# Alisah-Ozcan/HEonGPU

Hardware: AMD Instinct MI355X
Metric: homomorphic mults/sec (CKKS N=2^16, L=16) + NTT GB/s vs HBM roofline (higher is better)
Workload: dtype u64

## Files before the change

heongpu_amd/csrc/ntt.hip:

```cpp
#include "ntt.hpp"
#define HEGPU_FP_TU ntt
#include "fpmod.cuh"

namespace hegpu {

#define NTT_THREADS 256

#ifdef NTT_ABLATION_HEADER
#include NTT_ABLATION_HEADER
#else
__device__ __forceinline__ u64 gld(const u64* p) { return *p; }
__device__ __forceinline__ void gst(u64* p, u64 v) { *p = v; }
#define NTT_ABLATE_BFLY(x, y, w)
#define NTT_ABLATE_FPBFLY(x, y, w)
#define NTT_ABLATE_TW(load, root0, s) (load)
#define NTT_FP_TW(t, i, c) ((t)[i])
#endif

__device__ __forceinline__ u64 csub(u64 x, u64 m) { return (x >= m) ? x - m : x; }

typedef unsigned long long u64x2_t __attribute__((ext_vector_type(2)));
struct ConstTw {
    const u64x2_t __attribute__((address_space(4)))* p;
    __device__ __forceinline__ ulonglong2 operator[](u32 i) const
// ... 618 lines not shown
    for (int k = 0; k < 8; k++)
        *reinterpret_cast<ulonglong2*>(&lds[row_phys(row * 256 + 16 * i0 + 2 * k)]) =
            make_ulonglong2(x[2 * k], x[2 * k + 1]);
    wave_lds_fence();
    row_store_all(a, ps, md, a.out + ps.out_off, (u64) blockIdx.x * 4096 + row * 256 + i0, lds, row, i0);
}

__device__ __forceinline__ void fwd_row_body_fp(const NttArgs& a, const PolySel& ps, const Mod& md, u64* lds)
{
    const int t = threadIdx.x;
    const FC fc = make_fc(md.q, FP_SITE(FPS_FWD_ROW, a.n_power - 12));
    const int s1 = a.n_power - 8;
    const ulonglong2* __restrict__ tw = a.tw + ((u64) ps.mod << a.n_power);
    u64* __restrict__ p = a.out + ps.out_off + (u64) blockIdx.x * 4096;

    const int row = t >> 4, i0 = t & 15;
    const u32 crow = blockIdx.x * 16 + row;
    double x[16];
#pragma unroll
    for (int k = 0; k < 16; k++) x[k] = as_f64(p[row * 256 + i0 + 16 * k]);
    fp_ct_radix<4>(x, tw, (1u << s1) + crow, fc, 0u, true);
#pragma unroll
    for (int k = 0; k < 16; k++) lds[row_phys(row * 256 + i0 + 16 * k)] = as_bits(x[k]);
    wave_lds_fence();
#pragma unroll
    for (int k = 0; k < 8; k++) {
        ulonglong2 v = *reinterpret_cast<const ulonglong2*>(&lds[row_phys(row * 256 + 16 * i0 + 2 * k)]);
        x[2 * k] = as_f64(v.x);
        x[2 * k + 1] = as_f64(v.y);
    }
    fp_ct_radix16_tb8(x, a.twB8 + ((u64) ps.mod * (15u << (a.n_power - 4))) + ((u64) crow * 15 * 16 + i0), fc);
    wave_lds_fence();
#pragma unroll
    for (int k = 0; k < 8; k++)
        *reinterpret_cast<ulonglong2*>(&lds[row_phys(row * 256 + 16 * i0 + 2 * k)]) =
            make_ulonglong2(fp_to_u64(x[2 * k]), fp_to_u64(x[2 * k + 1]));
    wave_lds_fence();
    row_store_all(a, ps, md, a.out + ps.out_off, (u64) blockIdx.x * 4096 + row * 256 + i0, lds, row, i0);
}

__global__ __launch_bounds__(NTT_THREADS) void ntt_fwd_row(NttArgs a)
{
    __shared__ __attribute__((aligned(16))) u64 lds[ROW_LDS_ELEMS];
    const PolySel ps = select_poly(a, blockIdx.y);
    if (a.skip_identity && ps.mod == ps.digit) return;
    const Mod md = a.mods[ps.mod];
    if (md.fp) fwd_row_body_fp(a, ps, md, lds);
    else if (row_stages_lazy(md, a.lazy_q_max)) fwd_row_body<true>(a, ps, md, lds);
    else fwd_row_body<false>(a, ps, md, lds);
}

template <int S1>
__device__ __forceinline__ int single_pos(int row, int col)
{
    return (row >> 4) * 4096 + row_phys((row & 15) * 256 + col);
}

template <int S1, bool FP, bool LAZY, bool DECOMP = false>
__device__ __forceinline__ void fwd_single_body(const NttArgs& a, const PolySel& ps, const Mod& md, u64* limb)
{
    constexpr int R = 1 << S1;
    constexpr int CT = 4096 / R;
    constexpr int NSA = S1 - 4;
    constexpr int RA = 1 << NSA;
    constexpr int G = 16 / RA;
    const int t = threadIdx.x, g = t >> 8, tt = t & 255;
    const QC qc = make_qc(md.q);
    const FC fc = make_fc(md.q, FP_SITE(FPS_FWD_SINGLE, S1 - 4));
    const ulonglong2* __restrict__ tw = a.tw + ((u64) ps.mod << a.n_power);
    const u64* __restrict__ src = a.in + ps.in_off + g * CT;
    const int col = tt % CT, r1 = tt / CT;
    u64 dv[DECOMP ? 16 : 1];
    double dy[(DECOMP && FP) ? 16 : 1];
    if constexpr (DECOMP) {
        if constexpr (NSA > 0) {
#pragma unroll
            for (int gi = 0; gi < G; gi++) {
                const int L = tt + 256 * gi;
                const int c = L % CT, rb = L / CT;
#pragma unroll
                for (int k = 0; k < RA; k++) dv[gi * RA + k] = src[(u64) (rb + 16 * k) * 256 + c];
            }
        } else {
#pragma unroll
            for (int k = 0; k < 16; k++) dv[k] = src[(u64) k * 256 + col];
        }
        const u64 half_qP = a.half_on ? a.mods[a.half_src_mod].q : 0;
        if constexpr (FP) {
            FP_STAGE(fc, FP_STAGE_INPUT);
            if (a.half_on) {
#pragma unroll
                for (int k = 0; k < 16; k++) dv[k] = add_mod(dv[k], a.half, half_qP);
            }
            if (a.mods[a.half_on ? a.half_src_mod : ps.digit].bit > 52) {
                const double c32 = (double) reduce64(1ull << 32, md), c32i = c32 * fc.qi;
#pragma unroll
                for (int k = 0; k < 16; k++)
                    dy[k] = fp_mul(fp_from_u32((u32) (dv[k] >> 32)), c32, c32i, fc) + fp_from_u32((u32) dv[k]);
            } else {
#pragma unroll
                for (int k = 0; k < 16; k++) dy[k] = fp_reduce(fp_from_u64(dv[k]), fc);
            }
            if (a.half_on) {
                const double half_hm = fp_from_u64(a.half_mod[ps.mod]);
#pragma unroll
                for (int k = 0; k < 16; k++) dy[k] = fp_reduce(dy[k] - half_hm, fc);
            }
#pragma unroll
            for (int k = 0; k < 16; k++) FP_AUDIT_VAL(fc, FPM_SUM, dy[k]);
        } else {
            if (a.half_on) {
                const u64 half_hm = a.half_mod[ps.mod];
#pragma unroll
                for (int k = 0; k < 16; k++) dv[k] = sub_mod(reduce64(add_mod(dv[k], a.half, half_qP), md), half_hm, md.q);
            } else if (!LAZY && a.mods[ps.digit].q > 8 * md.q) {
#pragma unroll
                for (int k = 0; k < 16; k++) dv[k] = reduce64(dv[k], md);
            }
        }
    }
    if constexpr (FP) {
        double x[16];
        if constexpr (NSA > 0) {
#pragma unroll
            for (int gi = 0; gi < G; gi++) {
                const int L = tt + 256 * gi;
                const int c = L % CT, rb = L / CT;
                double y[RA];
#pragma unroll
                for (int k = 0; k < RA; k++) {
                    if constexpr (DECOMP) y[k] = dy[gi * RA + k];
                    else y[k] = fp_from_u64(gld(&src[(u64) (rb + 16 * k) * 256 + c]));
                }
                fp_ct_radix<NSA>(y, tw, 1u, fc, FpColSched<S1>::a_before, false);
#pragma unroll
                for (int k = 0; k < RA; k++) limb[single_pos<S1>(rb + 16 * k, g * CT + c)] = as_bits(y[k]);
            }
            __syncthreads();
#pragma unroll
            for (int k = 0; k < 16; k++) x[k] = as_f64(limb[single_pos<S1>(16 * r1 + k, g * CT + col)]);
        } else {
#pragma unroll
            for (int k = 0; k < 16; k++) {
                if constexpr (DECOMP) x[k] = dy[k];
                else x[k] = fp_from_u64(src[(u64) k * 256 + col]);
            }
        }
        fp_ct_radix<4>(x, tw, (u32) (RA + r1), fc, FpColSched<S1>::b_before, FpColSched<S1>::b_at_end);
#pragma unroll
        for (int k = 0; k < 16; k++) limb[single_pos<S1>(16 * r1 + k, g * CT + col)] = as_bits(x[k]);
    } else {
        u64 x[16];
        if constexpr (NSA > 0) {
#pragma unroll
            for (int gi = 0; gi < G; gi++) {
                const int L = tt + 256 * gi;
                const int c = L % CT, rb = L / CT;
                u64 y[RA];
#pragma unroll
                for (int k = 0; k < RA; k++) {
                    if constexpr (DECOMP) y[k] = dv[gi * RA + k];
                    else y[k] = gld(&src[(u64) (rb + 16 * k) * 256 + c]);
                }
                ct_radix<NSA, LAZY>(y, tw, 1u, qc);
#pragma unroll
                for (int k = 0; k < RA; k++) limb[single_pos<S1>(rb + 16 * k, g * CT + c)] = y[k];
            }
            __syncthreads();
#pragma unroll
            for (int k = 0; k < 16; k++) x[k] = limb[single_pos<S1>(16 * r1 + k, g * CT + col)];
        } else {
#pragma unroll
            for (int k = 0; k < 16; k++) {
                if constexpr (DECOMP) x[k] = dv[k];
                else x[k] = src[(u64) k * 256 + col];
            }
        }
        ct_radix<4, LAZY>(x, tw, (u32) (RA + r1), qc);
#pragma unroll
        for (int k = 0; k < 16; k++) limb[single_pos<S1>(16 * r1 + k, g * CT + col)] = x[k];
    }
    __syncthreads();
    u64* lds = limb + g * 4096;
    const int row = tt >> 4, i0 = tt & 15;
    const u32 crow = g * 16 + row;
    const ulonglong2* __restrict__ tb = a.twB + ((u64) ps.mod * (15u << (a.n_power - 4))) + ((u64) crow * 15 * 16 + i0);
    u64 r[16];
    if constexpr (FP) {
        double x[16];
#pragma unroll
        for (int k = 0; k < 16; k++) x[k] = as_f64(lds[row_phys(row * 256 + i0 + 16 * k)]);
        fp_ct_radix<4>(x, tw, (1u << S1) + crow, fc, 0u, true);
#pragma unroll
        for (int k = 0; k < 16; k++) lds[row_phys(row * 256 + i0 + 16 * k)] = as_bits(x[k]);
        wave_lds_fence();
#pragma unroll
        for (int k = 0; k < 8; k++) {
            ulonglong2 v = *reinterpret_cast<const ulonglong2*>(&lds[row_phys(row * 256 + 16 * i0 + 2 * k)]);
            x[2 * k] = as_f64(v.x);
            x[2 * k + 1] = as_f64(v.y);
        }
        fp_ct_radix16_tb8(x, a.twB8 + ((u64) ps.mod * (15u << (a.n_power - 4))) + ((u64) crow * 15 * 16 + i0), fc);
#pragma unroll
        for (int k = 0; k < 16; k++) r[k] = fp_to_u64(x[k]);
    } else {
        u64 x[16];
#pragma unroll
        for (int k = 0; k < 16; k++) x[k] = lds[row_phys(row * 256 + i0 + 16 * k)];
        ct_radix<4, LAZY>(x, tw, (1u << S1) + crow, qc);
#pragma unroll
        for (int k = 0; k < 16; k++) lds[row_phys(row * 256 + i0 + 16 * k)] = x[k];
        wave_lds_fence();
#pragma unroll
        for (int k = 0; k < 8; k++) {
            ulonglong2 v = *reinterpret_cast<const ulonglong2*>(&lds[row_phys(row * 256 + 16 * i0 + 2 * k)]);
            x[2 * k] = v.x;
            x[2 * k + 1] = v.y;
        }
        ct_radix16_tb<LAZY>(x, tb, qc);
        if (LAZY) {
#pragma unroll
            for (int k = 0; k < 16; k++) r[k] = reduce64(x[k], md);
        } else {
#pragma unroll
            for (int k = 0; k < 16; k++) r[k] = csub(csub(csub(x[k], qc.q4), 2 * qc.q), qc.q);
        }
    }
    wave_lds_fence();
#pragma unroll
    for (int k = 0; k < 8; k++)
        *reinterpret_cast<ulonglong2*>(&lds[row_phys(row * 256 + 16 * i0 + 2 * k)]) = make_ulonglong2(r[2 * k], r[2 * k + 1]);
    wave_lds_fence();
    row_store_all(a, ps, md, a.out + ps.out_off, (u64) g * 4096 + row * 256 + i0, lds, row, i0);
}

template <int S1, bool DECOMP = false>
__global__ __launch_bounds__(16 << S1, 4) void ntt_fwd_single(NttArgs a)
{
    extern __shared__ __attribute__((aligned(16))) u64 limb[];
    const PolySel ps = select_poly(a, blockIdx.x);
    if (DECOMP && a.skip_identity && ps.mod == ps.digit) return;
    const Mod md = a.mods[ps.mod];
    if (md.fp) fwd_single_body<S1, true, false, DECOMP>(a, ps, md, limb);
    else if (fwd_stages_lazy(md, a.lazy_q_max)) fwd_single_body<S1, false, true, DECOMP>(a, ps, md, limb);
    else fwd_single_body<S1, false, false, DECOMP>(a, ps, md, limb);
}

__device__ __forceinline__ void acc128(u64& hi, u64& lo, u64 a, u64 b)
{
    u64 h, l;
    mul64wide(a, b, h, l);
    lo += l;
    hi += h + (lo < l);
}

template <bool LAZY>
__device__ __forceinline__ void ks_row_digit(u64 (&x)[16], const u64* __restrict__ p, u64* lds,
                                             const ulonglong2* twa, const ulonglong2* __restrict__ tb,
                                             const QC& qc, const Mod& md, int row, int i0)
{
#pragma unroll
    for (int k = 0; k < 16; k++) x[k] = gld(&p[row * 256 + i0 + 16 * k]);
#pragma unroll
    for (int s = 0; s < 4; s++) {
        const int half = 8 >> s;
#pragma unroll
        for (int b = 0; b < (1 << s); b++) {
            const ulonglong2 w = twa[((1 << s) - 1 + b) * 16 + row];
#pragma unroll
            for (int j = 0; j < half; j++) ct_bfly<LAZY>(x[b * 2 * half + j], x[b * 2 * half + j + half], w, qc);
        }
    }
#pragma unroll
    for (int k = 0; k < 16; k++) lds[row_phys(row * 256 + i0 + 16 * k)] = x[k];
    wave_lds_fence();
#pragma unroll
    for (int k = 0; k < 8; k++) {
        ulonglong2 v = *reinterpret_cast<const ulonglong2*>(&lds[row_phys(row * 256 + 16 * i0 + 2 * k)]);
        x[2 * k] = v.x;
        x[2 * k + 1] = v.y;
    }
    ct_radix16_tb<LAZY>(x, tb, qc);
    if (!LAZY) {
#pragma unroll
        for (int k = 0; k < 16; k++) x[k] = csub(csub(csub(x[k], qc.q4), 2 * qc.q), qc.q);
    }
    wave_lds_fence();
#pragma unroll
    for (int k = 0; k < 8; k++)
        *reinterpret_cast<ulonglong2*>(&lds[row_phys(row * 256 + 16 * i0 + 2 * k)]) =
            make_ulonglong2(x[2 * k], x[2 * k + 1]);
    wave_lds_fence();
#pragma unroll
    for (int k = 0; k < 16; k++) x[k] = lds[row_phys(row * 256 + i0 + 16 * k)];
    wave_lds_fence();
}

struct KsIdx { int item, tile, slot; bool valid; int d0, d1; };
__host__ __device__ __forceinline__ unsigned ks_slots(const KsMacArgs& a, int kind)
{
    if (a.int_slot_count <= 0 || kind == 0) return (unsigned) a.rc;
    return kind == 1 ? (unsigned) a.int_slot_count : (unsigned) (a.rc - a.int_slot_count);
}
template <bool SPLIT, int KIND = 0>
__device__ __forceinline__ KsIdx ks_index(const KsMacArgs& a)
{
    const unsigned b = blockIdx.x, xcd = b & 7u, j = b >> 3;
    const unsigned splits = SPLIT ? (unsigned) a.splits : 1u;
    const unsigned units = (unsigned) a.items * splits;
    const unsigned tiles = 1u << (a.n_power - 12);
    const unsigned total = ks_slots(a, KIND) * tiles * units, chunk = (total + 7u) >> 3;
    const unsigned lin = xcd * chunk + j;
    const unsigned g = lin / units, unit = lin - g * units;
    const unsigned item = SPLIT ? unit / splits : unit, sp = SPLIT ? unit - item * splits : 0u;
    const unsigned nslots = ks_slots(a, KIND), gt = g / nslots;
    KsIdx r;
    r.valid = lin < total;
    r.item = (int) item;
    r.tile = (int) gt;
    int si = (int) (g - gt * nslots);
    if (KIND == 1 && a.int_slot_count > 0) {
        si = a.int_slots[r.valid ? si : 0];
    } else if (KIND == 2 && a.int_slot_count > 0) {
#pragma unroll
        for (int q = 0; q < 8; q++)
            if (q < a.int_slot_count && a.int_slots[q] <= si) si++;
    }
    r.slot = si;
    r.d0 = SPLIT ? (int) (sp * (unsigned) a.digits / splits) : 0;
    r.d1 = SPLIT ? (int) ((sp + 1) * (unsigned) a.digits / splits) : a.digits;
    return r;
}

#define KS_TW_LDS_BYTES ((15 * 256 + 15 * 16) * 8)
template <bool SPLIT>
__device__ __forceinline__ void ks_row_mac_int_body(const KsMacArgs& a, const KsIdx& ki, const Mod& md, int midx,
                                                    u64* lds, void* twbuf)
{
    const int t = threadIdx.x;
    const int item = ki.item, tile = ki.tile, slot = ki.slot;
    const QC qc = make_qc(md.q);
    const int s1 = a.n_power - 8;
    const ulonglong2* __restrict__ tw = a.tw + ((u64) midx << a.n_power);
    const int row = t >> 4, i0 = t & 15;
    const u32 crow = tile * 16 + row;
    const ulonglong2* __restrict__ tb = a.twB + ((u64) midx * (15u << (a.n_power - 4))) + ((u64) crow * 15 * 16 + i0);
    const u64 n = (u64) 1 << a.n_power;
    const u64* __restrict__ pin = a.in + a.in_item_stride * item + ((u64) slot << a.n_power) + (u64) tile * 4096;
    const u64* __restrict__ pk = a.key + ((u64) midx << a.n_power) + (u64) tile * 4096 + row * 256 + i0;
    const u64 dig_off = (u64) a.rc << a.n_power;
    const u64 key_off1 = (u64) a.key_limbs << a.n_power, key_off2 = (u64) a.key_limbs << (a.n_power + 1);
    const bool lazy = row_stages_lazy(md, a.lazy_q_max) && md.q <= ~0ull / (u64) a.digits;
    ulonglong2* twa = reinterpret_cast<ulonglong2*>(twbuf);
    if (i0 < 15) {
        const int s = (i0 >= 7) ? 3 : (i0 >= 3) ? 2 : (i0 >= 1) ? 1 : 0;
        twa[i0 * 16 + row] = tw[((((u32) 1 << s1) + crow) << s) + (i0 - ((1 << s) - 1))];
    }
    wave_lds_fence();

    u64 h0[16], l0[16], h1[16], l1[16];
#pragma unroll
    for (int k = 0; k < 16; k++) h0[k] = l0[k] = h1[k] = l1[k] = 0;
    for (int i = ki.d0; i < ki.d1; i++) {
        u64 x[16];
        const u64* p = pin + dig_off * i;
        if (a.skip_identity && i == midx) {
            const u64* pi = a.ident + a.ident_item_stride * item + ((u64) i << a.n_power) + (u64) tile * 4096;
#pragma unroll
            for (int k = 0; k < 16; k++) x[k] = gld(&pi[row * 256 + i0 + 16 * k]);
        } else if (lazy) {
            ks_row_digit<true>(x, p, lds, twa, tb, qc, md, row, i0);
        } else {
            ks_row_digit<false>(x, p, lds, twa, tb, qc, md, row, i0);
        }
        const u64* k0 = pk + key_off2 * i;
        const u64* k1 = k0 + key_off1;
#pragma unroll
        for (int k = 0; k < 16; k++) {
            acc128(h0[k], l0[k], x[k], k0[16 * k]);
            acc128(h1[k], l1[k], x[k], k1[16 * k]);
        }
    }
    u64* po = (SPLIT ? const_cast<u64*>(pin) + dig_off * ki.d0 - (u64) tile * 4096
                     : a.out + a.out_item_stride * item + ((u64) slot << a.n_power)) +
              (u64) tile * 4096 + row * 256 + i0;
#pragma unroll
    for (int k = 0; k < 16; k++) {
        po[16 * k] = reduce128(h0[k], l0[k], md);
        po[dig_off + 16 * k] = reduce128(h1[k], l1[k], md);
    }
    (void) n;
}

template <bool SPLIT>
__global__ __launch_bounds__(NTT_THREADS, SPLIT ? 2 : 1) void ks_row_mac(KsMacArgs a)
{
    __shared__ __attribute__((aligned(16))) u64 lds[ROW_LDS_ELEMS];
    __shared__ ulonglong2 twa[15 * 16];
    const KsIdx ki = ks_index<SPLIT, SPLIT ? 0 : 1>(a);
    if (!ki.valid) return;
    const int midx = a.mod_order ? a.mod_order[ki.slot] : ki.slot;
    const Mod md = a.mods[midx];
    if (md.fp) return;
    ks_row_mac_int_body<SPLIT>(a, ki, md, midx, lds, twa);
}

template <bool SPLIT>
__device__ __forceinline__ void ks_row_mac_fp_body(const KsMacArgs& a, const KsIdx& ki, const Mod& md, int midx,
                                                   u64* lds, void* twbuf)
{
    const int t = threadIdx.x;
    const int item = ki.item, tile = ki.tile, slot = ki.slot;
    const FC fc = make_fc(md.q, FP_SITE(SPLIT ? FPS_KS_ROW_SPLIT : FPS_KS_ROW, a.n_power - 12));
    const int s1 = a.n_power - 8;
    const ulonglong2* __restrict__ tw = a.tw + ((u64) midx << a.n_power);
    const int row = t >> 4, i0 = t & 15;
    const u32 crow = tile * 16 + row;
    const double* __restrict__ tb8 = a.twB8 + ((u64) midx * (15u << (a.n_power - 4))) + ((u64) crow * 15 * 16 + i0);
    const u64* __restrict__ pin = a.in + a.in_item_stride * item + ((u64) slot << a.n_power) + (u64) tile * 4096;
    const u64* __restrict__ pk = a.key + ((u64) midx << a.n_power) + (u64) tile * 4096 + row * 256 + i0;
    const u64 dig_off = (u64) a.rc << a.n_power;
    const u64 key_off1 = (u64) a.key_limbs << a.n_power, key_off2 = (u64) a.key_limbs << (a.n_power + 1);

    double* twl = reinterpret_cast<double*>(twbuf);
#pragma unroll
    for (int k = 0; k < 15; k++) twl[k * 256 + t] = tb8[k * 16];
    if (i0 < 15) {
        const int s = (i0 >= 7) ? 3 : (i0 >= 3) ? 2 : (i0 >= 1) ? 1 : 0;
        const int b = i0 - ((1 << s) - 1);
        twl[15 * 256 + i0 * 16 + row] = as_f64(tw[((((u32) 1 << s1) + crow) << s) + b].x);
    }
    wave_lds_fence();

    double a0[16], a1[16];
#pragma unroll
    for (int k = 0; k < 16; k++) a0[k] = a1[k] = 0.0;
    int since = 0;
    for (int i = ki.d0; i < ki.d1; i++) {
        double x[16];
        const u64* p = pin + dig_off * i;
        const bool ident = a.skip_identity && i == midx;
        const u64* px = ident ? a.ident + a.ident_item_stride * item + ((u64) i << a.n_power) + (u64) tile * 4096 : p;
        u64 xr[16];
#pragma unroll
        for (int k = 0; k < 16; k++) {
            if constexpr (!SPLIT) xr[k] = __builtin_nontemporal_load(&px[row * 256 + i0 + 16 * k]);
            else xr[k] = px[row * 256 + i0 + 16 * k];
        }
        const u64* k0 = pk + key_off2 * i;
        const u64* k1 = k0 + key_off1;
        u64 kv0[16], kv1[16];
#pragma unroll
        for (int k = 0; k < 16; k++) {
            kv0[k] = k0[16 * k];
            kv1[k] = k1[16 * k];
        }
        if (ident) {
            FP_STAGE(fc, FP_STAGE_INPUT);
#pragma unroll
            for (int k = 0; k < 16; k++) x[k] = fp_reduce(fp_from_u64(xr[k]), fc);
        } else {
            if constexpr (SPLIT) {
#pragma unroll
                for (int k = 0; k < 16; k++) x[k] = as_f64(xr[k]);
#pragma unroll
                for (int s = 0; s < 4; s++) {
                    const int half = 8 >> s;
                    FP_STAGE(fc, s1 + s);
#pragma unroll
                    for (int b = 0; b < (1 << s); b++) {
                        const double w = twl[15 * 256 + ((1 << s) - 1 + b) * 16 + row];
                        const ulonglong2 wp = make_ulonglong2(as_bits(w), as_bits(w * fc.qi));
#pragma unroll
                        for (int j = 0; j < half; j++) fp_ct_bfly(x[b * 2 * half + j], x[b * 2 * half + j + half], wp, fc);
                    }
                }
                FP_STAGE(fc, s1 + 4);
#pragma unroll
                for (int k = 0; k < 16; k++) x[k] = fp_reduce(x[k], fc);
#pragma unroll
                for (int k = 0; k < 16; k++) lds[row_phys(row * 256 + i0 + 16 * k)] = as_bits(x[k]);
                wave_lds_fence();
#pragma unroll
                for (int k = 0; k < 8; k++) {
                    ulonglong2 v = *reinterpret_cast<const ulonglong2*>(&lds[row_phys(row * 256 + 16 * i0 + 2 * k)]);
                    x[2 * k] = as_f64(v.x);
                    x[2 * k + 1] = as_f64(v.y);
                }
#pragma unroll
                for (int s = 0; s < 4; s++) {
                    const int half = 8 >> s;
                    FP_STAGE(fc, s1 + 4 + s);
#pragma unroll
                    for (int b = 0; b < (1 << s); b++) {
                        const double wd = twl[((1 << s) - 1 + b) * 256 + t];
                        const ulonglong2 w = make_ulonglong2(as_bits(wd), as_bits(wd * fc.qi));
#pragma unroll
                        for (int j = 0; j < half; j++) fp_ct_bfly(x[b * 2 * half + j], x[b * 2 * half + j + half], w, fc);
                    }
                }
            } else {
                int row_o = row, t_o = t;
                asm volatile("" : "+v"(row_o), "+v"(t_o));
                const double* twa = twl + 15 * 256 + row_o;
                const double* twb = twl + t_o;
                double wn[8], wc[8];
                wc[0] = twa[0];
                wn[0] = twa[16];
                wn[1] = twa[32];
                __builtin_amdgcn_sched_barrier(0);
#pragma unroll
                for (int k = 0; k < 16; k++) x[k] = as_f64(xr[k]);
#pragma unroll
                for (int s = 0; s < 4; s++) {
                    const int half = 8 >> s;
                    FP_STAGE(fc, s1 + s);
                    if (s > 0) {
#pragma unroll
                        for (int b = 0; b < (1 << s); b++) wc[b] = wn[b];
                    }
                    if (s < 3) {
                        if (s > 0) {
#pragma unroll
                            for (int b = 0; b < (2 << s); b++) wn[b] = twa[((2 << s) - 1 + b) * 16];
                        }
                    } else {
                        wn[0] = twb[0];
                    }
                    __builtin_amdgcn_sched_barrier(0);
#pragma unroll
                    for (int b = 0; b < (1 << s); b++) {
                        const double w = wc[b];
                        const ulonglong2 wp = make_ulonglong2(as_bits(w), as_bits(w * fc.qi));
#pragma unroll
                        for (int j = 0; j < half; j++) fp_ct_bfly(x[b * 2 * half + j], x[b * 2 * half + j + half], wp, fc);
                    }
                }
                FP_STAGE(fc, s1 + 4);
#pragma unroll
                for (int k = 0; k < 16; k++) x[k] = fp_reduce(x[k], fc);
#pragma unroll
                for (int k = 0; k < 16; k++) lds[row_phys(row * 256 + i0 + 16 * k)] = as_bits(x[k]);
                wave_lds_fence();
#pragma unroll
                for (int k = 0; k < 8; k++) {
                    ulonglong2 v = *reinterpret_cast<const ulonglong2*>(&lds[row_phys(row * 256 + 16 * i0 + 2 * k)]);
                    x[2 * k] = as_f64(v.x);
                    x[2 * k + 1] = as_f64(v.y);
                }
#pragma unroll
                for (int s = 0; s < 4; s++) {
                    const int half = 8 >> s;
                    FP_STAGE(fc, s1 + 4 + s);
#pragma unroll
                    for (int b = 0; b < (1 << s); b++) wc[b] = wn[b];
                    if (s < 3) {
#pragma unroll
                        for (int b = 0; b < (2 << s); b++) wn[b] = twb[((2 << s) - 1 + b) * 256];
                    }
                    __builtin_amdgcn_sched_barrier(0);
#pragma unroll
                    for (int b = 0; b < (1 << s); b++) {
                        const double wd = wc[b];
                        const ulonglong2 w = make_ulonglong2(as_bits(wd), as_bits(wd * fc.qi));
#pragma unroll
                        for (int j = 0; j < half; j++) fp_ct_bfly(x[b * 2 * half + j], x[b * 2 * half + j + half], w, fc);
                    }
                }
            }
            wave_lds_fence();
#pragma unroll
            for (int k = 0; k < 8; k++)
                *reinterpret_cast<ulonglong2*>(&lds[row_phys(row * 256 + 16 * i0 + 2 * k)]) =
                    make_ulonglong2(as_bits(x[2 * k]), as_bits(x[2 * k + 1]));
            wave_lds_fence();
#pragma unroll
            for (int k = 0; k < 16; k++) x[k] = as_f64(lds[row_phys(row * 256 + i0 + 16 * k)]);
            wave_lds_fence();
        }
#pragma unroll
        for (int k = 0; k < 16; k++) {
            const double xi = x[k] * fc.qi;
            FP_STAGE(fc, FP_STAGE_PRODUCT);
            a0[k] += fp_mul(fp_from_u64(kv0[k]), x[k], xi, fc);
            a1[k] += fp_mul(fp_from_u64(kv1[k]), x[k], xi, fc);
            FP_STAGE(fc, FP_STAGE_SUMS + since);
            FP_AUDIT_VAL(fc, FPM_SUM, a0[k]);
            FP_AUDIT_VAL(fc, FPM_SUM, a1[k]);
        }
        if (++since == 3) {
            since = 0;
            FP_STAGE(fc, FP_STAGE_SUMS + 3);
#pragma unroll
            for (int k = 0; k < 16; k++) {
                a0[k] = fp_reduce(a0[k], fc);
                a1[k] = fp_reduce(a1[k], fc);
            }
        }
    }
    u64* po = (SPLIT ? const_cast<u64*>(pin) + dig_off * ki.d0 - (u64) tile * 4096
                     : a.out + a.out_item_stride * item + ((u64) slot << a.n_power)) +
              (u64) tile * 4096 + row * 256 + i0;
    FP_STAGE(fc, FP_STAGE_OUT);
#pragma unroll
    for (int k = 0; k < 16; k++) {
        if constexpr (!SPLIT) {
            __builtin_nontemporal_store(fp_to_u64(fp_canon(a0[k], fc)), &po[16 * k]);
            __builtin_nontemporal_store(fp_to_u64(fp_canon(a1[k], fc)), &po[dig_off + 16 * k]);
        } else {
            po[16 * k] = fp_to_u64(fp_canon(a0[k], fc));
            po[dig_off + 16 * k] = fp_to_u64(fp_canon(a1[k], fc));
        }
    }
}

template <bool SPLIT>
__global__ __launch_bounds__(NTT_THREADS) void ks_row_mac_fp(KsMacArgs a)
{
    __shared__ __attribute__((aligned(16))) u64 lds[ROW_LDS_ELEMS];
    __shared__ double twl[15 * 256 + 15 * 16];
    const KsIdx ki = ks_index<SPLIT, SPLIT ? 0 : 2>(a);
    if (!ki.valid) return;
    const int midx = a.mod_order ? a.mod_order[ki.slot] : ki.slot;
    const Mod md = a.mods[midx];
    if (!md.fp) return;
    ks_row_mac_fp_body<SPLIT>(a, ki, md, midx, lds, twl);
}

__global__ __launch_bounds__(NTT_THREADS, 2) void ks_row_mac_split(KsMacArgs a)
{
    __shared__ __attribute__((aligned(16))) u64 lds[ROW_LDS_ELEMS];
    __shared__ double twl[15 * 256 + 15 * 16];
    const KsIdx ki = ks_index<true>(a);
    if (!ki.valid) return;
    const int midx = a.mod_order ? a.mod_order[ki.slot] : ki.slot;
    const Mod md = a.mods[midx];
    if (md.fp) ks_row_mac_fp_body<true>(a, ki, md, midx, lds, twl);
    else ks_row_mac_int_body<true>(a, ki, md, midx, lds, twl);
}

hipError_t ks_row_mac_launch(const KsMacArgs& a, int items, hipStream_t st)
{
    if (a.digits > 64 || items <= 0) return hipErrorInvalidValue;
    if (a.splits > 1 && a.digits < 2 * a.splits) return hipErrorInvalidValue;
    KsMacArgs k = a;
    k.items = items;
    if (k.int_slot_count < 0 || k.int_slot_count > 8) k.int_slot_count = 0;
    const unsigned tiles = (1u << a.n_power) / 4096, units = (unsigned) items * (a.splits > 1 ? (unsigned) a.splits : 1u);
    auto grid_of = [&](int kind) { return dim3(8u * ((ks_slots(k, kind) * tiles * units + 7u) / 8u)); };
    if (a.splits > 1) {
        hipLaunchKernelGGL(ks_row_mac_split, grid_of(0), dim3(NTT_THREADS), 0, st, k);
    } else {
        if (!a.no_fp && ks_slots(k, 2) > 0)
            hipLaunchKernelGGL(ks_row_mac_fp<false>, grid_of(2), dim3(NTT_THREADS), 0, st, k);
        if (!a.no_int && ks_slots(k, 1) > 0)
            hipLaunchKernelGGL(ks_row_mac<false>, grid_of(1), dim3(NTT_THREADS), 0, st, k);
    }
    return hipGetLastError();
}

__device__ __forceinline__ void fp_gs_bfly(double& x, double& y, ulonglong2 w, const FC& c)
{
    const double s = x + y, d = x - y;
    x = s;
    y = fp_mul(d, as_f64(w.x), as_f64(w.y), c);
    FP_AUDIT_VAL(c, FPM_SUM, s);
}

struct ArInt {
    typedef u64 T;
    QC qc;
    __device__ __forceinline__ explicit ArInt(const Mod& md) : qc(make_qc(md.q)) {}
    __device__ __forceinline__ T from_canon(u64 v) const { return v; }
    __device__ __forceinline__ T from_bits(u64 v) const { return v; }
    __device__ __forceinline__ u64 to_bits(T v) const { return v; }
    template <int LOGR>
    __device__ __forceinline__ void radix(T (&x)[1 << LOGR], const ulonglong2* __restrict__ tw, u32 root0) const
    {
        gs_radix<LOGR>(x, tw, root0, qc);
    }
    __device__ __forceinline__ void radix16_tb(T (&x)[16], const ulonglong2* __restrict__ tb) const { gs_radix16_tb(x, tb, qc); }
    template <int LOGR>
    __device__ __forceinline__ void radix_last(T (&x)[1 << LOGR], const ulonglong2* __restrict__ tw, ulonglong2 ninv,
                                               ulonglong2 w1ninv, u64 (&out)[1 << LOGR]) const
    {
        gs_radix_last<LOGR>(x, tw, 1u, ninv, w1ninv, qc);
#pragma unroll
        for (int k = 0; k < (1 << LOGR); k++) out[k] = x[k];
    }
};

struct ArFp {
    typedef double T;
    FC fc;
    int s1;
    __device__ __forceinline__ explicit ArFp(const Mod& md, int n_power) : fc(make_fc(md.q, FP_SITE(FPS_INV, n_power - 12))), s1(n_power - 8) {}
    __device__ __forceinline__ T from_canon(u64 v) const { return fp_from_u64(v); }
    __device__ __forceinline__ T from_bits(u64 v) const { return as_f64(v); }
    __device__ __forceinline__ u64 to_bits(T v) const { return as_bits(v); }
    template <int N>
    __device__ __forceinline__ void reduce_all(T (&x)[N]) const
    {
#pragma unroll
        for (int k = 0; k < N; k++) x[k] = fp_reduce(x[k], fc);
    }
    template <int LOGR>
    __device__ __forceinline__ void radix(T (&x)[1 << LOGR], const ulonglong2* __restrict__ tw, u32 root0) const
    {
        int done = 0;
#pragma unroll
        for (int s = LOGR - 1; s >= 0; s--) {
            const int half = (1 << LOGR) >> (s + 1);
            FP_STAGE(fc, 31 - __builtin_clz(root0) + s);
#pragma unroll
            for (int b = 0; b < (1 << s); b++) {
                const ulonglong2 w = tw[(root0 << s) + b];
#pragma unroll
                for (int j = 0; j < half; j++) fp_gs_bfly(x[b * 2 * half + j], x[b * 2 * half + j + half], w, fc);
            }
            if ((++done & 1) == 0 || s == 0) reduce_all(x);
        }
    }
    __device__ __forceinline__ void radix16_tb(T (&x)[16], const ulonglong2* __restrict__ tb) const
    {
#pragma unroll
        for (int s = 3; s >= 0; s--) {
            const int half = 8 >> s;
            FP_STAGE(fc, s1 + 4 + s);
#pragma unroll
            for (int b = 0; b < (1 << s); b++) {
                const ulonglong2 w = tb[((1 << s) - 1 + b) * 16];
#pragma unroll
                for (int j = 0; j < half; j++) fp_gs_bfly(x[b * 2 * half + j], x[b * 2 * half + j + half], w, fc);
            }
            if (s == 2 || s == 0) reduce_all(x);
        }
    }
    template <int LOGR>
    __device__ __forceinline__ void radix_last(T (&x)[1 << LOGR], const ulonglong2* __restrict__ tw, ulonglong2 ninv,
                                               ulonglong2 w1ninv, u64 (&out)[1 << LOGR]) const
    {
        int done = 0;
#pragma unroll
        for (int s = LOGR - 1; s >= 1; s--) {
            const int half = (1 << LOGR) >> (s + 1);
            FP_STAGE(fc, s);
#pragma unroll
            for (int b = 0; b < (1 << s); b++) {
                const ulonglong2 w = tw[(1u << s) + b];
#pragma unroll
                for (int j = 0; j < half; j++) fp_gs_bfly(x[b * 2 * half + j], x[b * 2 * half + j + half], w, fc);
            }
            if ((++done & 1) == 0) reduce_all(x);
        }
        constexpr int half = (1 << LOGR) >> 1;
        FP_STAGE(fc, 0);
#pragma unroll
        for (int j = 0; j < half; j++) {
            const double sum = x[j] + x[j + half], d = x[j] - x[j + half];
            out[j] = fp_to_u64(fp_canon(fp_mul(sum, as_f64(ninv.x), as_f64(ninv.y), fc), fc));
            out[j + half] = fp_to_u64(fp_canon(fp_mul(d, as_f64(w1ninv.x), as_f64(w1ninv.y), fc), fc));
        }
    }
};

template <typename AR, bool TO_LDS, bool TENSOR = false>
__device__ __forceinline__ void inv_row_part(const AR& ar, const NttArgs& a, int mod, int tt, u32 crow0,
                                             const u64* __restrict__ src, u64* __restrict__ dst, u64* lds,
                                             int tensor_part = 0)
{
    typedef typename AR::T T;
    const int s1 = a.n_power - 8;
    const ulonglong2* __restrict__ tw = a.itw + ((u64) mod << a.n_power);
    const int row = tt >> 4, i0 = tt & 15;
    const u32 crow = crow0 + row;
    if (TENSOR) {
        const Mod md = a.mods[mod];
        const u64 part_off = (u64) a.tensor_limbs << a.n_power;
        const u64* __restrict__ a0 = src, * __restrict__ a1 = src + part_off, * __restrict__ b0 = src + 2 * part_off,
                 * __restrict__ b1 = src + 3 * part_off;
#pragma unroll
        for (int k0 = 0; k0 < 16; k0 += 4) {
            u64 r[4];
            if (tensor_part == 1) {
                u64 va0[4], va1[4], vb0[4], vb1[4];
#pragma unroll
                for (int k = 0; k < 4; k++) {
                    const int e = row * 256 + i0 + 16 * (k0 + k);
                    va0[k] = a0[e]; va1[k] = a1[e]; vb0[k] = b0[e]; vb1[k] = b1[e];
                }
#pragma unroll
                for (int k = 0; k < 4; k++) {
                    u64 h1, l1, h2, l2;
                    mul64wide(va0[k], vb1[k], h1, l1);
                    mul64wide(va1[k], vb0[k], h2, l2);
                    const u64 lo = l1 + l2;
                    r[k] = reduce128(h1 + h2 + (lo < l1), lo, md);
                }
            } else {
                const u64* __restrict__ pa = tensor_part == 0 ? a0 : a1;
                const u64* __restrict__ pb = tensor_part == 0 ? b0 : b1;
                u64 va[4], vb[4];
#pragma unroll
                for (int k = 0; k < 4; k++) {
                    const int e = row * 256 + i0 + 16 * (k0 + k);
                    va[k] = pa[e]; vb[k] = pb[e];
                }
#pragma unroll
                for (int k = 0; k < 4; k++) r[k] = mul_barrett(va[k], vb[k], md);
            }
#pragma unroll
            for (int k = 0; k < 4; k++) lds[row_phys(row * 256 + i0 + 16 * (k0 + k))] = r[k];
        }
    } else {
#pragma unroll
        for (int k = 0; k < 16; k++) lds[row_phys(row * 256 + i0 + 16 * k)] = gld(&src[row * 256 + i0 + 16 * k]);
    }
    wave_lds_fence();
    T x[16];
#pragma unroll
    for (int k = 0; k < 8; k++) {
        ulonglong2 v = *reinterpret_cast<const ulonglong2*>(&lds[row_phys(row * 256 + 16 * i0 + 2 * k)]);
        x[2 * k] = ar.from_canon(v.x);
        x[2 * k + 1] = ar.from_canon(v.y);
    }
    ar.radix16_tb(x, a.itwB + ((u64) mod * (15u << (a.n_power - 4))) + ((u64) crow * 15 * 16 + i0));
    wave_lds_fence();
#pragma unroll
    for (int k = 0; k < 8; k++)
        *reinterpret_cast<ulonglong2*>(&lds[row_phys(row * 256 + 16 * i0 + 2 * k)]) =
            make_ulonglong2(ar.to_bits(x[2 * k]), ar.to_bits(x[2 * k + 1]));
    wave_lds_fence();
#pragma unroll
    for (int k = 0; k < 16; k++) x[k] = ar.from_bits(lds[row_phys(row * 256 + i0 + 16 * k)]);
    ar.template radix<4>(x, tw, (1u << s1) + crow);
    if constexpr (TO_LDS) {
#pragma unroll
        for (int k = 0; k < 16; k++) lds[row_phys(row * 256 + i0 + 16 * k)] = ar.to_bits(x[k]);
    } else {
#pragma unroll
        for (int k = 0; k < 16; k++) gst(&dst[row * 256 + i0 + 16 * k], ar.to_bits(x[k]));
    }
}

struct InvEpi {
    const u64* last;
    const u64* ct;
    u64* out;
    Mod md;
    u64 half, qP, hm, inv;
    int galois, n_power;
    bool pre;
};
__device__ __forceinline__ bool inv_epi_setup(const NttArgs& a, const PolySel& ps, InvEpi& e, bool& skip)
{
    skip = false;
    if (!a.iepi.on) return false;
    const NttInvEpilogue& ep = a.iepi;
    const int pc = ep.p_count ? ep.p_count : 1;
    const int part = udiv16(ps.j, ep.mg_slots), limb = ps.j - part * (ep.limbs + pc);
    if (limb >= ep.limbs) { skip = true; return true; }
    const u64 item_in = a.out_item_stride * ps.item;
    const u64 off = (u64) (part * ep.limbs + limb) << a.n_power;
    e.pre = ep.u != nullptr;
    e.last = e.pre ? ep.u + ep.u_item_stride * ps.item + off
                   : a.out + item_in + ((u64) (part * (ep.limbs + 1) + ep.limbs) << a.n_power);
    e.ct = (ep.ct && part < ep.add_parts) ? ep.ct + ep.ct_item_stride * ps.item + off : nullptr;
    e.out = ep.out + ep.out_item_stride * ps.item + off;
    e.md = a.mods[ps.mod];
    e.half = ep.half;
    e.qP = a.mods[ep.p_mod].q;
    e.hm = e.pre ? 0 : ep.half_mod[limb];
    e.inv = ep.inv[limb];
    e.galois = ep.galois_elt;
    e.n_power = a.n_power;
    return true;
}
template <int CNT, bool EPI, typename POS>
__device__ __forceinline__ void inv_store(const InvEpi& epr, u64* __restrict__ p, u32 e0, POS pos, const u64 (&o)[CNT])
{
    if constexpr (!EPI) {
#pragma unroll
        for (int k = 0; k < CNT; k++) gst(&p[pos(k)], o[k]);
        return;
    }
    const InvEpi* ep = &epr;
    u64 lv[CNT], cv[CNT], r[CNT];
#pragma unroll
    for (int k = 0; k < CNT; k++) lv[k] = ep->last[e0 + pos(k)];
    if (ep->ct) {
#pragma unroll
        for (int k = 0; k < CNT; k++) cv[k] = ep->ct[e0 + pos(k)];
    }
    if (!ep->pre) {
#pragma unroll
        for (int k = 0; k < CNT; k++) {
            u64 l = add_mod(lv[k], ep->half, ep->qP);
            l = reduce64(l, ep->md);
            lv[k] = sub_mod(l, ep->hm, ep->md.q);
        }
    }
#pragma unroll
    for (int k = 0; k < CNT; k++) r[k] = mul_barrett(sub_mod(o[k], lv[k], ep->md.q), ep->inv, ep->md);
    if (ep->ct) {
#pragma unroll
        for (int k = 0; k < CNT; k++) r[k] = add_mod(cv[k], r[k], ep->md.q);
    }
    if (ep->galois) {
#pragma unroll
        for (int k = 0; k < CNT; k++) {
            const u32 raw = (e0 + (u32) pos(k)) * (u32) ep->galois;
            ep->out[raw & ((1u << ep->n_power) - 1u)] = ((raw >> ep->n_power) & 1u) ? ep->md.q - r[k] : r[k];
        }
    } else {
#pragma unroll
        for (int k = 0; k < CNT; k++) ep->out[e0 + pos(k)] = r[k];
    }
}

template <int S1, typename AR, bool FROM_LDS, bool KEEP = false, bool EPI = false>
__device__ __forceinline__ void inv_col_part(const AR& ar, const NttArgs& a, int mod, int tt, int g, u64* __restrict__ p,
                                             u64* buf, u64 (&keep)[16], const InvEpi& ep = InvEpi(), u32 e0 = 0)
{
    typedef typename AR::T T;
    constexpr int R = 1 << S1;
    constexpr int CT = 4096 / R;
    constexpr int NSA = S1 - 4;
    constexpr int RA = 1 << NSA;
    constexpr int G = 16 / RA;
    const ulonglong2* __restrict__ tw = a.itw + ((u64) mod << a.n_power);
    const ulonglong2 ninv = a.ninv[mod], w1ninv = a.w1ninv[mod];
    const int col = tt % CT, r1 = tt / CT;
    auto pos = [&](int row, int c) -> int {
        if constexpr (FROM_LDS) return single_pos<S1>(row, g * CT + c);
        else return col_phys(row * CT + c);
    };
    T x[16];
#pragma unroll
    for (int k = 0; k < 16; k++)
        x[k] = ar.from_bits(FROM_LDS ? buf[pos(16 * r1 + k, col)] : gld(&p[(u64) (16 * r1 + k) * 256 + col]));
    if constexpr (NSA > 0) {
        ar.template radix<4>(x, tw, (u32) (RA + r1));
#pragma unroll
        for (int k = 0; k < 16; k++) buf[pos(16 * r1 + k, col)] = ar.to_bits(x[k]);
        __syncthreads();
#pragma unroll
        for (int gi = 0; gi < G; gi++) {
            const int L = tt + NTT_THREADS * gi;
            const int c = L % CT, rb = L / CT;
            T y[RA];
            u64 o[RA];
#pragma unroll
            for (int k = 0; k < RA; k++) y[k] = ar.from_bits(buf[pos(rb + 16 * k, c)]);
            ar.template radix_last<NSA>(y, tw, ninv, w1ninv, o);
            if constexpr (RA == 16) {
                u64 oa[8], ob[8];
#pragma unroll
                for (int k = 0; k < 8; k++) { oa[k] = o[k]; ob[k] = o[8 + k]; }
                inv_store<8, EPI>(ep, p, e0, [&](int k) { return (u32) ((rb + 16 * k) * 256 + c); }, oa);
// ... 443 lines not shown
```

Baseline: 8002.

## Rework FP key-switch row MAC to 2048-element tiles with 8 values per thread

The non-split FP key-switch MAC kernel now processes 2048-element tiles as 8 rows of 256, with each thread holding 8 values instead of 16. It runs the 8 butterfly stages in three register groups joined by padded LDS transposes, and uses a smaller twiddle table in LDS. Launch bounds are raised to allow 4 blocks per CU. The aim is to cut register and LDS pressure so more waves are resident to hide HBM latency. The cost is more LDS round-trips and barriers per digit, a doubled block count, and new swizzle index functions that must be exactly right.

Result: no change. 8105 (median of 6 runs) (+1.3%).

```diff
diff --git a/heongpu_amd/csrc/ntt.hip b/heongpu_amd/csrc/ntt.hip
--- a/heongpu_amd/csrc/ntt.hip
+++ b/heongpu_amd/csrc/ntt.hip
@@ -944,13 +944,13 @@
     if (a.int_slot_count <= 0 || kind == 0) return (unsigned) a.rc;
     return kind == 1 ? (unsigned) a.int_slot_count : (unsigned) (a.rc - a.int_slot_count);
 }
-template <bool SPLIT, int KIND = 0>
+template <bool SPLIT, int KIND = 0, int TILE_LOG = 12>
 __device__ __forceinline__ KsIdx ks_index(const KsMacArgs& a)
 {
     const unsigned b = blockIdx.x, xcd = b & 7u, j = b >> 3;
     const unsigned splits = SPLIT ? (unsigned) a.splits : 1u;
     const unsigned units = (unsigned) a.items * splits;
-    const unsigned tiles = 1u << (a.n_power - 12);
+    const unsigned tiles = 1u << (a.n_power - TILE_LOG);
     const unsigned total = ks_slots(a, KIND) * tiles * units, chunk = (total + 7u) >> 3;
     const unsigned lin = xcd * chunk + j;
     const unsigned g = lin / units, unit = lin - g * units;
@@ -1047,13 +1047,12 @@
     ks_row_mac_int_body<SPLIT>(a, ki, md, midx, lds, twa);
 }
 
-template <bool SPLIT>
-__device__ __forceinline__ void ks_row_mac_fp_body(const KsMacArgs& a, const KsIdx& ki, const Mod& md, int midx,
-                                                   u64* lds, void* twbuf)
+__device__ __forceinline__ void ks_row_mac_fp_split_body(const KsMacArgs& a, const KsIdx& ki, const Mod& md, int midx,
+                                                         u64* lds, void* twbuf)
 {
     const int t = threadIdx.x;
     const int item = ki.item, tile = ki.tile, slot = ki.slot;
-    const FC fc = make_fc(md.q, FP_SITE(SPLIT ? FPS_KS_ROW_SPLIT : FPS_KS_ROW, a.n_power - 12));
+    const FC fc = make_fc(md.q, FP_SITE(FPS_KS_ROW_SPLIT, a.n_power - 12));
     const int s1 = a.n_power - 8;
     const ulonglong2* __restrict__ tw = a.tw + ((u64) midx << a.n_power);
     const int row = t >> 4, i0 = t & 15;
@@ -1085,10 +1084,7 @@
         const u64* px = ident ? a.ident + a.ident_item_stride * item + ((u64) i << a.n_power) + (u64) tile * 4096 : p;
         u64 xr[16];
 #pragma unroll
-        for (int k = 0; k < 16; k++) {
-            if constexpr (!SPLIT) xr[k] = __builtin_nontemporal_load(&px[row * 256 + i0 + 16 * k]);
-            else xr[k] = px[row * 256 + i0 + 16 * k];
-        }
+        for (int k = 0; k < 16; k++) xr[k] = px[row * 256 + i0 + 16 * k];
         const u64* k0 = pk + key_off2 * i;
         const u64* k1 = k0 + key_off1;
         u64 kv0[16], kv1[16];
@@ -1102,112 +1098,42 @@
 #pragma unroll
             for (int k = 0; k < 16; k++) x[k] = fp_reduce(fp_from_u64(xr[k]), fc);
         } else {
-            if constexpr (SPLIT) {
-#pragma unroll
-                for (int k = 0; k < 16; k++) x[k] = as_f64(xr[k]);
-#pragma unroll
-                for (int s = 0; s < 4; s++) {
-                    const int half = 8 >> s;
-                    FP_STAGE(fc, s1 + s);
-#pragma unroll
-                    for (int b = 0; b < (1 << s); b++) {
-                        const double w = twl[15 * 256 + ((1 << s) - 1 + b) * 16 + row];
-                        const ulonglong2 wp = make_ulonglong2(as_bits(w), as_bits(w * fc.qi));
-#pragma unroll
-                        for (int j = 0; j < half; j++) fp_ct_bfly(x[b * 2 * half + j], x[b * 2 * half + j + half], wp, fc);
-                    }
+#pragma unroll
+            for (int k = 0; k < 16; k++) x[k] = as_f64(xr[k]);
+#pragma unroll
+            for (int s = 0; s < 4; s++) {
+                const int half = 8 >> s;
+                FP_STAGE(fc, s1 + s);
+#pragma unroll
+                for (int b = 0; b < (1 << s); b++) {
+                    const double w = twl[15 * 256 + ((1 << s) - 1 + b) * 16 + row];
+                    const ulonglong2 wp = make_ulonglong2(as_bits(w), as_bits(w * fc.qi));
+#pragma unroll
+                    for (int j = 0; j < half; j++) fp_ct_bfly(x[b * 2 * half + j], x[b * 2 * half + j + half], wp, fc);
                 }
-                FP_STAGE(fc, s1 + 4);
-#pragma unroll
-                for (int k = 0; k < 16; k++) x[k] = fp_reduce(x[k], fc);
-#pragma unroll
-                for (int k = 0; k < 16; k++) lds[row_phys(row * 256 + i0 + 16 * k)] = as_bits(x[k]);
-                wave_lds_fence();
-#pragma unroll
-                for (int k = 0; k < 8; k++) {
-                    ulonglong2 v = *reinterpret_cast<const ulonglong2*>(&lds[row_phys(row * 256 + 16 * i0 + 2 * k)]);
-                    x[2 * k] = as_f64(v.x);
-                    x[2 * k + 1] = as_f64(v.y);
-                }
-#pragma unroll
-                for (int s = 0; s < 4; s++) {
-                    const int half = 8 >> s;
-                    FP_STAGE(fc, s1 + 4 + s);
-#pragma unroll
-                    for (int b = 0; b < (1 << s); b++) {
-                        const double wd = twl[((1 << s) - 1 + b) * 256 + t];
-                        const ulonglong2 w = make_ulonglong2(as_bits(wd), as_bits(wd * fc.qi));
-#pragma unroll
-                        for (int j = 0; j < half; j++) fp_ct_bfly(x[b * 2 * half + j], x[b * 2 * half + j + half], w, fc);
-                    }
-                }
-            } else {
-                int row_o = row, t_o = t;
-                asm volatile("" : "+v"(row_o), "+v"(t_o));
-                const double* twa = twl + 15 * 256 + row_o;
-                const double* twb = twl + t_o;
-                double wn[8], wc[8];
-                wc[0] = twa[0];
-                wn[0] = twa[16];
-                wn[1] = twa[32];
-                __builtin_amdgcn_sched_barrier(0);
-#pragma unroll
-                for (int k = 0; k < 16; k++) x[k] = as_f64(xr[k]);
-#pragma unroll
-                for (int s = 0; s < 4; s++) {
-                    const int half = 8 >> s;
-                    FP_STAGE(fc, s1 + s);
-                    if (s > 0) {
-#pragma unroll
-                        for (int b = 0; b < (1 << s); b++) wc[b] = wn[b];
-                    }
-                    if (s < 3) {
-                        if (s > 0) {
-#pragma unroll
-                            for (int b = 0; b < (2 << s); b++) wn[b] = twa[((2 << s) - 1 + b) * 16];
-                        }
-                    } else {
-                        wn[0] = twb[0];
-                    }
-                    __builtin_amdgcn_sched_barrier(0);
-#pragma unroll
-                    for (int b = 0; b < (1 << s); b++) {
-                        const double w = wc[b];
-                        const ulonglong2 wp = make_ulonglong2(as_bits(w), as_bits(w * fc.qi));
-#pragma unroll
-                        for (int j = 0; j < half; j++) fp_ct_bfly(x[b * 2 * half + j], x[b * 2 * half + j + half], wp, fc);
-                    }
-                }
-                FP_STAGE(fc, s1 + 4);
-#pragma unroll
-                for (int k = 0; k < 16; k++) x[k] = fp_reduce(x[k], fc);
-#pragma unroll
-                for (int k = 0; k < 16; k++) lds[row_phys(row * 256 + i0 + 16 * k)] = as_bits(x[k]);
-                wave_lds_fence();
-#pragma unroll
-                for (int k = 0; k < 8; k++) {
-                    ulonglong2 v = *reinterpret_cast<const ulonglong2*>(&lds[row_phys(row * 256 + 16 * i0 + 2 * k)]);
-                    x[2 * k] = as_f64(v.x);
-                    x[2 * k + 1] = as_f64(v.y);
-                }
-#pragma unroll
-                for (int s = 0; s < 4; s++) {
-                    const int half = 8 >> s;
-                    FP_STAGE(fc, s1 + 4 + s);
-#pragma unroll
-                    for (int b = 0; b < (1 << s); b++) wc[b] = wn[b];
-                    if (s < 3) {
-#pragma unroll
-                        for (int b = 0; b < (2 << s); b++) wn[b] = twb[((2 << s) - 1 + b) * 256];
-                    }
-                    __builtin_amdgcn_sched_barrier(0);
-#pragma unroll
-                    for (int b = 0; b < (1 << s); b++) {
-                        const double wd = wc[b];
-                        const ulonglong2 w = make_ulonglong2(as_bits(wd), as_bits(wd * fc.qi));
-#pragma unroll
-                        for (int j = 0; j < half; j++) fp_ct_bfly(x[b * 2 * half + j], x[b * 2 * half + j + half], w, fc);
-                    }
+            }
+            FP_STAGE(fc, s1 + 4);
+#pragma unroll
+            for (int k = 0; k < 16; k++) x[k] = fp_reduce(x[k], fc);
+#pragma unroll
+            for (int k = 0; k < 16; k++) lds[row_phys(row * 256 + i0 + 16 * k)] = as_bits(x[k]);
+            wave_lds_fence();
+#pragma unroll
+            for (int k = 0; k < 8; k++) {
+                ulonglong2 v = *reinterpret_cast<const ulonglong2*>(&lds[row_phys(row * 256 + 16 * i0 + 2 * k)]);
+                x[2 * k] = as_f64(v.x);
+                x[2 * k + 1] = as_f64(v.y);
+            }
+#pragma unroll
+            for (int s = 0; s < 4; s++) {
+                const int half = 8 >> s;
+                FP_STAGE(fc, s1 + 4 + s);
+#pragma unroll
+                for (int b = 0; b < (1 << s); b++) {
+                    const double wd = twl[((1 << s) - 1 + b) * 256 + t];
+                    const ulonglong2 w = make_ulonglong2(as_bits(wd), as_bits(wd * fc.qi));
+#pragma unroll
+                    for (int j = 0; j < half; j++) fp_ct_bfly(x[b * 2 * half + j], x[b * 2 * half + j + half], w, fc);
                 }
             }
             wave_lds_fence();
@@ -1240,33 +1166,204 @@
             }
         }
     }
-    u64* po = (SPLIT ? const_cast<u64*>(pin) + dig_off * ki.d0 - (u64) tile * 4096
-                     : a.out + a.out_item_stride * item + ((u64) slot << a.n_power)) +
-              (u64) tile * 4096 + row * 256 + i0;
+    u64* po = const_cast<u64*>(pin) + dig_off * ki.d0 + row * 256 + i0;
     FP_STAGE(fc, FP_STAGE_OUT);
 #pragma unroll
     for (int k = 0; k < 16; k++) {
-        if constexpr (!SPLIT) {
-            __builtin_nontemporal_store(fp_to_u64(fp_canon(a0[k], fc)), &po[16 * k]);
-            __builtin_nontemporal_store(fp_to_u64(fp_canon(a1[k], fc)), &po[dig_off + 16 * k]);
+        po[16 * k] = fp_to_u64(fp_canon(a0[k], fc));
+        po[dig_off + 16 * k] = fp_to_u64(fp_canon(a1[k], fc));
+    }
+}
+
+#define KS8_TILE_LOG 11
+#define KS8_TILE (1 << KS8_TILE_LOG)
+#define KS8_TWC 0
+#define KS8_TWB (6 * 256)
+#define KS8_TWA (KS8_TWB + 8 * 7 * 8)
+#define KS8_TW_DOUBLES (KS8_TWA + 8 * 7)
+#define KS8_ROW_STRIDE 284
+__host__ __device__ constexpr int ks8_ab(int e) { return (e & 31) + 36 * (e >> 5); }
+__host__ __device__ constexpr int ks8_bc(int e) { return (e >> 5) + 8 * ((e >> 3) & 3) + 36 * (e & 7); }
+__host__ __device__ constexpr int ks8_ca(int e) { return (e & 31) + 33 * (e >> 5); }
+__host__ __device__ constexpr int ks8_cgrp(int j) { return (j & 1) | (((j >> 4) & 1) << 1) | (((j >> 1) & 7) << 2); }
+
+__device__ __forceinline__ void ks_row_mac_fp8_body(const KsMacArgs& a, const KsIdx& ki, const Mod& md, int midx,
+                                                    u64* lds, double* twl)
+{
+    const int t = threadIdx.x;
+    const int item = ki.item, tile = ki.tile, slot = ki.slot;
+    FC fc = make_fc(md.q, FP_SITE(FPS_KS_ROW, a.n_power - 12));
+    auto uniform = [](double v) {
+        const u64 b = as_bits(v);
+        return as_f64(((u64) __builtin_amdgcn_readfirstlane((u32) (b >> 32)) << 32) | (u32) __builtin_amdgcn_readfirstlane((u32) b));
+    };
+    fc.q = uniform(fc.q);
+    fc.qi = uniform(fc.qi);
+    const int s1 = a.n_power - 8;
+    const ulonglong2* __restrict__ tw = a.tw + ((u64) midx << a.n_power);
+    const int row = t >> 5, j = t & 31;
+    const int lo = row * 256 + j;
+    const u32 crow = tile * 8 + row;
+    const u64 tile_off = (u64) tile * KS8_TILE;
+    const u64* __restrict__ pin = a.in + a.in_item_stride * item + ((u64) slot << a.n_power) + tile_off;
+    const u64* __restrict__ pk = a.key + ((u64) midx << a.n_power) + tile_off;
+    const u64 dig_off = (u64) a.rc << a.n_power;
+    const u64 key_off1 = (u64) a.key_limbs << a.n_power, key_off2 = (u64) a.key_limbs << (a.n_power + 1);
+
+    const u32 root = ((u32) 1 << s1) + crow;
+    auto twv = [&](int s, int b) { return as_f64(tw[(root << s) + b].x); };
+#pragma unroll
+    for (int c = 0; c < 6; c++) twl[KS8_TWC + c * 256 + t] = c < 2 ? twv(6, 2 * ks8_cgrp(j) + c) : twv(7, 4 * ks8_cgrp(j) + c - 2);
+#pragma unroll
+    for (int h = 0; h < 2; h++) {
+        const int idx = j + 32 * h;
+        if (idx < 56) {
+            const int sl = idx >> 3, bk = idx & 7, sp = sl >= 3 ? 2 : sl >= 1 ? 1 : 0;
+            twl[KS8_TWB + row * 56 + idx] = twv(3 + sp, (bk << sp) + sl - ((1 << sp) - 1));
+        }
+    }
+    if (j < 7) {
+        const int sp = j >= 3 ? 2 : j >= 1 ? 1 : 0;
+        twl[KS8_TWA + row * 7 + j] = twv(sp, j - ((1 << sp) - 1));
+    }
+    wave_lds_fence();
+
+    const int xa = row * KS8_ROW_STRIDE + j, eb = 32 * (j >> 2) + (j & 3), ec = 8 * ks8_cgrp(j);
+    const int xb_ab = row * KS8_ROW_STRIDE + ks8_ab(eb), xb_bc = row * KS8_ROW_STRIDE + ks8_bc(eb);
+    const int xc_bc = row * KS8_ROW_STRIDE + ks8_bc(ec), xc_ca = row * KS8_ROW_STRIDE + ks8_ca(ec);
+
+    double a0[8], a1[8];
+#pragma unroll
+    for (int k = 0; k < 8; k++) a0[k] = a1[k] = 0.0;
+    int since = 0;
+    for (int i = ki.d0; i < ki.d1; i++) {
+        double x[8];
+        const bool ident = a.skip_identity && i == midx;
+        const u64* px = ident ? a.ident + a.ident_item_stride * item + ((u64) i << a.n_power) + tile_off : pin + dig_off * i;
+        u64 xr[8];
+#pragma unroll
+        for (int k = 0; k < 8; k++) xr[k] = __builtin_nontemporal_load(&px[lo + 32 * k]);
+        const u64* k0 = pk + key_off2 * i;
+        const u64* k1 = k0 + key_off1;
+        u64 kv0[8], kv1[8];
+#pragma unroll
+        for (int k = 0; k < 8; k++) kv0[k] = k0[lo + 32 * k];
+        auto load_kv1 = [&]() {
+#pragma unroll
+            for (int k = 0; k < 8; k++) kv1[k] = k1[lo + 32 * k];
+        };
+        if (ident) {
+            load_kv1();
+            FP_STAGE(fc, FP_STAGE_INPUT);
+#pragma unroll
+            for (int k = 0; k < 8; k++) x[k] = fp_reduce(fp_from_u64(xr[k]), fc);
         } else {
-            po[16 * k] = fp_to_u64(fp_canon(a0[k], fc));
-            po[dig_off + 16 * k] = fp_to_u64(fp_canon(a1[k], fc));
-        }
+            int th = t;
+            asm volatile("" : "+v"(th));
+            const int rw = th >> 5, bl = (th & 31) >> 2;
+            const int oa = KS8_TWA + rw * 7, ob = KS8_TWB + rw * 56 + bl, oc = KS8_TWC + th;
+            auto tws = [&](int s, int b) {
+                return s < 3 ? twl[oa + (1 << s) - 1 + b] : s < 6 ? twl[ob + ((1 << (s - 3)) - 1 + b) * 8]
+                                                                  : twl[oc + ((1 << (s - 5)) - 2 + b) * 256];
+            };
+            double wn[4], wc[4];
+            wc[0] = tws(0, 0);
+            wn[0] = tws(1, 0);
+            wn[1] = tws(1, 1);
+            __builtin_amdgcn_sched_barrier(0);
+#pragma unroll
+            for (int k = 0; k < 8; k++) x[k] = as_f64(xr[k]);
+#pragma unroll
+            for (int s = 0; s < 8; s++) {
+                if (s == 3) {
+#pragma unroll
+                    for (int k = 0; k < 8; k++) lds[xa + ks8_ab(32 * k)] = as_bits(x[k]);
+                    wave_lds_fence();
+#pragma unroll
+                    for (int k = 0; k < 8; k++) x[k] = as_f64(lds[xb_ab + ks8_ab(4 * k)]);
+                } else if (s == 6) {
+                    wave_lds_fence();
+#pragma unroll
+                    for (int k = 0; k < 8; k++) lds[xb_bc + ks8_bc(4 * k)] = as_bits(x[k]);
+                    wave_lds_fence();
+#pragma unroll
+                    for (int k = 0; k < 8; k++) x[k] = as_f64(lds[xc_bc + ks8_bc(k)]);
+                }
+                const int sr = s < 3 ? s : s < 6 ? s - 3 : s - 5;
+                const int half = 4 >> sr;
+                FP_STAGE(fc, s1 + s);
+                if (s == 4) {
+#pragma unroll
+                    for (int k = 0; k < 8; k++) x[k] = fp_reduce(x[k], fc);
+                }
+                if (s > 0) {
+#pragma unroll
+                    for (int b = 0; b < (1 << sr); b++) wc[b] = wn[b];
+                }
+                if (s > 0 && s < 7) {
+                    const int sn = s + 1, srn = sn < 3 ? sn : sn < 6 ? sn - 3 : sn - 5;
+#pragma unroll
+                    for (int b = 0; b < (1 << srn); b++) wn[b] = tws(sn, b);
+                }
+                __builtin_amdgcn_sched_barrier(0);
+#pragma unroll
+                for (int b = 0; b < (1 << sr); b++) {
+                    const double w = wc[b];
+                    const ulonglong2 wp = make_ulonglong2(as_bits(w), as_bits(w * fc.qi));
+#pragma unroll
+                    for (int h = 0; h < half; h++) fp_ct_bfly(x[b * 2 * half + h], x[b * 2 * half + h + half], wp, fc);
+                }
+            }
+            load_kv1();
+            wave_lds_fence();
+#pragma unroll
+            for (int k = 0; k < 8; k++) lds[xc_ca + ks8_ca(k)] = as_bits(x[k]);
+            wave_lds_fence();
+#pragma unroll
+            for (int k = 0; k < 8; k++) x[k] = as_f64(lds[xa + ks8_ca(32 * k)]);
+            wave_lds_fence();
+        }
+#pragma unroll
+        for (int k = 0; k < 8; k++) {
+            const double xi = x[k] * fc.qi;
+            FP_STAGE(fc, FP_STAGE_PRODUCT);
+            a0[k] += fp_mul(fp_from_u64(kv0[k]), x[k], xi, fc);
+            a1[k] += fp_mul(fp_from_u64(kv1[k]), x[k], xi, fc);
+            FP_STAGE(fc, FP_STAGE_SUMS + since);
+            FP_AUDIT_VAL(fc, FPM_SUM, a0[k]);
+            FP_AUDIT_VAL(fc, FPM_SUM, a1[k]);
+        }
+        if (++since == 3) {
+            since = 0;
+            FP_STAGE(fc, FP_STAGE_SUMS + 3);
+#pragma unroll
+            for (int k = 0; k < 8; k++) {
+                a0[k] = fp_reduce(a0[k], fc);
+                a1[k] = fp_reduce(a1[k], fc);
+            }
+        }
+    }
+    u64* po = a.out + a.out_item_stride * item + ((u64) slot << a.n_power) + tile_off + lo;
+    FP_STAGE(fc, FP_STAGE_OUT);
+#pragma unroll
+    for (int k = 0; k < 8; k++) {
+        __builtin_nontemporal_store(fp_to_u64(fp_canon(a0[k], fc)), &po[32 * k]);
+        __builtin_nontemporal_store(fp_to_u64(fp_canon(a1[k], fc)), &po[dig_off + 32 * k]);
     }
 }
 
 template <bool SPLIT>
-__global__ __launch_bounds__(NTT_THREADS) void ks_row_mac_fp(KsMacArgs a)
-{
-    __shared__ __attribute__((aligned(16))) u64 lds[ROW_LDS_ELEMS];
-    __shared__ double twl[15 * 256 + 15 * 16];
-    const KsIdx ki = ks_index<SPLIT, SPLIT ? 0 : 2>(a);
+__global__ __launch_bounds__(NTT_THREADS, 4) void ks_row_mac_fp(KsMacArgs a)
+{
+    static_assert(!SPLIT, "small launches go through ks_row_mac_split");
+    __shared__ __attribute__((aligned(16))) u64 lds[8 * KS8_ROW_STRIDE];
+    __shared__ double twl[KS8_TW_DOUBLES];
+    const KsIdx ki = ks_index<false, 2, KS8_TILE_LOG>(a);
     if (!ki.valid) return;
     const int midx = a.mod_order ? a.mod_order[ki.slot] : ki.slot;
     const Mod md = a.mods[midx];
     if (!md.fp) return;
-    ks_row_mac_fp_body<SPLIT>(a, ki, md, midx, lds, twl);
+    ks_row_mac_fp8_body(a, ki, md, midx, lds, twl);
 }
 
 __global__ __launch_bounds__(NTT_THREADS, 2) void ks_row_mac_split(KsMacArgs a)
@@ -1277,7 +1374,7 @@
     if (!ki.valid) return;
     const int midx = a.mod_order ? a.mod_order[ki.slot] : ki.slot;
     const Mod md = a.mods[midx];
-    if (md.fp) ks_row_mac_fp_body<true>(a, ki, md, midx, lds, twl);
+    if (md.fp) ks_row_mac_fp_split_body(a, ki, md, midx, lds, twl);
     else ks_row_mac_int_body<true>(a, ki, md, midx, lds, twl);
 }
 
@@ -1288,15 +1385,17 @@
     KsMacArgs k = a;
     k.items = items;
     if (k.int_slot_count < 0 || k.int_slot_count > 8) k.int_slot_count = 0;
-    const unsigned tiles = (1u << a.n_power) / 4096, units = (unsigned) items * (a.splits > 1 ? (unsigned) a.splits : 1u);
-    auto grid_of = [&](int kind) { return dim3(8u * ((ks_slots(k, kind) * tiles * units + 7u) / 8u)); };
+    const unsigned units = (unsigned) items * (a.splits > 1 ? (unsigned) a.splits : 1u);
+    auto grid_of = [&](int kind, int tile_log) {
+        return dim3(8u * ((ks_slots(k, kind) * ((1u << a.n_power) >> tile_log) * units + 7u) / 8u));
+    };
     if (a.splits > 1) {
-        hipLaunchKernelGGL(ks_row_mac_split, grid_of(0), dim3(NTT_THREADS), 0, st, k);
+        hipLaunchKernelGGL(ks_row_mac_split, grid_of(0, 12), dim3(NTT_THREADS), 0, st, k);
     } else {
         if (!a.no_fp && ks_slots(k, 2) > 0)
-            hipLaunchKernelGGL(ks_row_mac_fp<false>, grid_of(2), dim3(NTT_THREADS), 0, st, k);
+            hipLaunchKernelGGL(ks_row_mac_fp<false>, grid_of(2, KS8_TILE_LOG), dim3(NTT_THREADS), 0, st, k);
         if (!a.no_int && ks_slots(k, 1) > 0)
-            hipLaunchKernelGGL(ks_row_mac<false>, grid_of(1), dim3(NTT_THREADS), 0, st, k);
+            hipLaunchKernelGGL(ks_row_mac<false>, grid_of(1, 12), dim3(NTT_THREADS), 0, st, k);
     }
     return hipGetLastError();
 }
```
